# sigp/consensus-specs

Measured on AMD Instinct MI355X. Metric: BLS sig verifications/sec (whole node), higher is better.
Workload: dtype u32 (381-bit Montgomery, 14x28-bit limbs in u32 words); 1 GPU; C2: 65536 independent bls_verify deposit PoP checks per GPU (domain=3, 1/16 tampered); global_batch=65536, parallelism=dp1 (independent items, no collective), batches_in_flight=1, subgroup_policy=pyecc

## Files before the change

consensus-specs_amd/csrc/bls381_defs.hpp:

```cpp
#pragma once
#include <stddef.h>
#include <stdint.h>

#if defined(__HIP__)
#include <hip/hip_runtime.h>
#if defined(__HIP_DEVICE_COMPILE__)
#define BLS_PHASE() __builtin_amdgcn_sched_barrier(0)
#define BLS_ANY(c) (__builtin_amdgcn_ballot_w64((c)) != 0)
#else
#define BLS_PHASE() ((void)0)
#define BLS_ANY(c) (c)
#endif
#define BLS_HD __host__ __device__
#define BLS_INLINE __host__ __device__ __forceinline__
#define BLS_NOINLINE __host__ __device__ __attribute__((noinline))
#define BLS_DEV_INLINE __host__ __device__ __forceinline__
#define BLS_CONST __device__ __constant__ static constexpr
#else
#define BLS_PHASE() ((void)0)
#define BLS_ANY(c) (c)
#define BLS_HD
#define BLS_INLINE inline __attribute__((always_inline))
#define BLS_NOINLINE __attribute__((noinline))
#define BLS_DEV_INLINE inline
#define BLS_CONST static constexpr
#endif

namespace bls381 {

constexpr int FP_LIMBS = 14;
constexpr int FP_BITS = 28;
constexpr uint32_t FP_MASK = (1u << 28) - 1;
struct fp_t { uint32_t w[14]; };
struct fp2_t { fp_t c0, c1; };
template <class E> struct fp6_g { E c0, c1, c2; };
template <class E> struct fp12_g { fp6_g<E> c0, c1; };
using fp6_t = fp6_g<fp2_t>;
using fp12_t = fp12_g<fp2_t>;
struct fp2p_t { fp_t v; };

struct g1_jac { fp_t x, y, z; };
struct g2_jac { fp2_t x, y, z; };
struct g1_aff { fp_t x, y; };
struct g2_aff { fp2_t x, y; };

constexpr int KBLOCK = 128;
struct agg_chunk { uint32_t begin, end; };
constexpr int ML_STEPS = 68;
constexpr int ML_LC = 5;
constexpr size_t ML_L_WORDS_PER_ITEM = (size_t)ML_STEPS * ML_LC * FP_LIMBS * 2;
enum : uint32_t { SSZ_CHUNK = 1, SSZ_MERKLE = 2 };
constexpr int SSZ_STACK = 64;
constexpr int SSZ_PROG_MAX = 512;

}
```

consensus-specs_amd/csrc/bls381_field.hpp:

```cpp
#pragma once
#include "bls381_defs.hpp"
#include "bls381_consts.hpp"

namespace bls381 {

#if defined(BLS_COUNT_OPS) && !defined(__HIP_DEVICE_COMPILE__)
inline thread_local uint64_t g_fp_macs = 0;
#define BLS_COUNT_MACS(k) (g_fp_macs += (k))
#else
#define BLS_COUNT_MACS(k) ((void)0)
#endif
#if !defined(__HIP_DEVICE_COMPILE__) && !defined(__HIP__)
inline uint64_t g_inv_fallbacks = 0;
#define BLS_COUNT_INV_FALLBACK() (++g_inv_fallbacks)
#else
#define BLS_COUNT_INV_FALLBACK() ((void)0)
#endif

BLS_INLINE fp_t fp_zero() { fp_t r; for (int i = 0; i < 14; ++i) r.w[i] = 0; return r; }
BLS_INLINE fp_t fp_one() { return FP_ONE_M; }

BLS_INLINE void fp_carry(int32_t (&t)[14]) {
#pragma unroll
  for (int i = 0; i < 13; ++i) {
    t[i + 1] += t[i] >> 28;
    t[i] &= (int32_t)FP_MASK;
  }
}

template <int KMAX>
BLS_INLINE fp_t fp_reduce_lc(const uint32_t (&s)[14]) {
  static_assert(KMAX >= 1 && KMAX <= 8, "value bound");
  int32_t t[14];
  if (KMAX <= 2) {
    const uint32_t m = (int32_t)s[13] > (int32_t)Q2_LIMBS[13] ? ~0u : 0u;
#pragma unroll
    for (int i = 0; i < 14; ++i) t[i] = (int32_t)(s[i] - (Q2_LIMBS[i] & m));
  } else {
    const int32_t top = (int32_t)s[13] > 0 ? (int32_t)s[13] : 0;
    const uint32_t k = (uint32_t)(((uint64_t)(uint32_t)top * LC_DIV_MAGIC) >> 40);
#pragma unroll
    for (int i = 0; i < 14; ++i) t[i] = (int32_t)(s[i] + k * NQ2_LIMBS[i]);
  }
  fp_carry(t);
  if (BLS_ANY(t[13] >= (int32_t)Q2_LIMBS[13])) {
    int32_t e[14];
#pragma unroll
    for (int i = 0; i < 14; ++i) e[i] = t[i] - (int32_t)Q2_LIMBS[i];
    fp_carry(e);
    const bool ge = e[13] >= 0;
#pragma unroll
    for (int i = 0; i < 14; ++i) t[i] = ge ? e[i] : t[i];
  }
  fp_t r;
#pragma unroll
  for (int i = 0; i < 14; ++i) r.w[i] = (uint32_t)t[i];
  return r;
}

BLS_INLINE fp_t fp_add(const fp_t& a, const fp_t& b) {
  uint32_t s[14];
#pragma unroll
  for (int i = 0; i < 14; ++i) s[i] = a.w[i] + b.w[i];
  return fp_reduce_lc<2>(s);
}

BLS_INLINE fp_t fp_sub(const fp_t& a, const fp_t& b) {
  uint32_t s[14];
#pragma unroll
  for (int i = 0; i < 14; ++i) s[i] = a.w[i] + Q2B_LIMBS[i] - b.w[i];
  return fp_reduce_lc<2>(s);
}

BLS_INLINE fp_t fp_neg(const fp_t& a) {
  uint32_t s[14];
#pragma unroll
  for (int i = 0; i < 14; ++i) s[i] = Q2B_LIMBS[i] - a.w[i];
  return fp_reduce_lc<2>(s);
}

BLS_INLINE fp_t fp_dbl(const fp_t& a) {
  uint32_t s[14];
#pragma unroll
  for (int i = 0; i < 14; ++i) s[i] = a.w[i] << 1;
  return fp_reduce_lc<2>(s);
}

BLS_INLINE fp_t fp_add_sub(const fp_t& a, const fp_t& b, const fp_t& c) {
  uint32_t s[14];
#pragma unroll
  for (int i = 0; i < 14; ++i) s[i] = a.w[i] + b.w[i] + Q2B_LIMBS[i] - c.w[i];
  return fp_reduce_lc<3>(s);
}

BLS_INLINE fp_t fp_add3(const fp_t& a, const fp_t& b, const fp_t& c) {
  uint32_t s[14];
#pragma unroll
  for (int i = 0; i < 14; ++i) s[i] = a.w[i] + b.w[i] + c.w[i];
  return fp_reduce_lc<3>(s);
}

BLS_INLINE fp_t fp_sub2(const fp_t& a, const fp_t& b, const fp_t& c) {
  uint32_t s[14];
#pragma unroll
  for (int i = 0; i < 14; ++i) s[i] = a.w[i] + Q4B_LIMBS[i] - b.w[i] - c.w[i];
  return fp_reduce_lc<3>(s);
}

BLS_INLINE fp_t fp_3m2(const fp_t& X, const fp_t& x) {
  uint32_t s[14];
#pragma unroll
  for (int i = 0; i < 14; ++i) s[i] = 3u * X.w[i] + Q4B_LIMBS[i] - (x.w[i] << 1);
  return fp_reduce_lc<5>(s);
}
BLS_INLINE fp_t fp_3p2(const fp_t& X, const fp_t& x) {
  uint32_t s[14];
#pragma unroll
  for (int i = 0; i < 14; ++i) s[i] = 3u * X.w[i] + (x.w[i] << 1);
  return fp_reduce_lc<5>(s);
}
BLS_INLINE fp_t fp_3pm2(const fp_t& X, const fp_t& x, bool minus) {
  uint32_t s[14];
#pragma unroll
  for (int i = 0; i < 14; ++i) {
    const uint32_t x2 = x.w[i] << 1;
    s[i] = 3u * X.w[i] + (minus ? Q4B_LIMBS[i] - x2 : x2);
  }
  return fp_reduce_lc<5>(s);
}

BLS_INLINE fp_t fp_add_lazy(const fp_t& a, const fp_t& b) {
  fp_t r;
#pragma unroll
  for (int i = 0; i < 14; ++i) r.w[i] = a.w[i] + b.w[i];
  return r;
}

BLS_INLINE fp_t fp_reduce_once(const fp_t& s) {
  int32_t b[14];
#pragma unroll
  for (int i = 0; i < 14; ++i) b[i] = (int32_t)s.w[i] - (int32_t)Q_LIMBS[i];
  fp_carry(b);
  const bool neg = b[13] < 0;
  fp_t r;
#pragma unroll
  for (int i = 0; i < 14; ++i) r.w[i] = neg ? s.w[i] : (uint32_t)b[i];
  return r;
}

BLS_INLINE bool fp_is_zero(const fp_t& a) {
  uint32_t z = 0, e = 0;
#pragma unroll
  for (int i = 0; i < 14; ++i) { z |= a.w[i]; e |= a.w[i] ^ Q_LIMBS[i]; }
  return z == 0 || e == 0;
}

BLS_INLINE bool fp_eq(const fp_t& a, const fp_t& b) { return fp_is_zero(fp_sub(a, b)); }

BLS_INLINE fp_t fp_half(const fp_t& a) {
  const uint32_t odd = a.w[0] & 1u;
  int32_t s[14];
#pragma unroll
  for (int i = 0; i < 14; ++i) s[i] = (int32_t)(a.w[i] + (odd ? Q_LIMBS[i] : 0u));
  fp_carry(s);
  fp_t r;
#pragma unroll
  for (int i = 0; i < 13; ++i) r.w[i] = ((uint32_t)s[i] >> 1) | (((uint32_t)s[i + 1] & 1u) << 27);
  r.w[13] = (uint32_t)s[13] >> 1;
  return r;
}

BLS_INLINE fp_t fp_mul_body(const fp_t& a, const fp_t& b) {
  uint64_t T[28];
#pragma unroll
  for (int k = 0; k < 28; ++k) T[k] = 0;
#pragma unroll
  for (int i = 0; i < 14; ++i)
#pragma unroll
    for (int j = 0; j < 14; ++j) T[i + j] += (uint64_t)a.w[i] * b.w[j];
#pragma unroll
  for (int i = 0; i < 14; ++i) {
    const uint32_t m = ((uint32_t)T[i] * Q_INV28) & FP_MASK;
#pragma unroll
    for (int j = 0; j < 14; ++j) T[i + j] += (uint64_t)m * Q_LIMBS[j];
    T[i + 1] += T[i] >> 28;
  }
  fp_t r;
  uint64_t c = 0;
#pragma unroll
  for (int j = 0; j < 14; ++j) {
    const uint64_t v = T[14 + j] + c;
    r.w[j] = (uint32_t)v & FP_MASK;
    c = v >> 28;
  }
  return r;
}

BLS_INLINE fp_t fp_sqr_body(const fp_t& a) {
  uint64_t T[28];
  uint32_t a2[14];
#pragma unroll
  for (int k = 0; k < 28; ++k) T[k] = 0;
#pragma unroll
  for (int i = 0; i < 14; ++i) a2[i] = a.w[i] << 1;
#pragma unroll
  for (int i = 0; i < 14; ++i) {
    T[2 * i] += (uint64_t)a.w[i] * a.w[i];
#pragma unroll
    for (int j = i + 1; j < 14; ++j) T[i + j] += (uint64_t)a2[i] * a.w[j];
  }
#pragma unroll
  for (int i = 0; i < 14; ++i) {
    const uint32_t m = ((uint32_t)T[i] * Q_INV28) & FP_MASK;
#pragma unroll
    for (int j = 0; j < 14; ++j) T[i + j] += (uint64_t)m * Q_LIMBS[j];
    T[i + 1] += T[i] >> 28;
  }
  fp_t r;
  uint64_t c = 0;
#pragma unroll
  for (int j = 0; j < 14; ++j) {
    const uint64_t v = T[14 + j] + c;
    r.w[j] = (uint32_t)v & FP_MASK;
    c = v >> 28;
  }
  return r;
}

#if defined(__clang__)
typedef uint32_t fpv_t __attribute__((ext_vector_type(14)));
BLS_INLINE fpv_t fp_pack(const fp_t& a) {
  fpv_t v;
#pragma unroll
  for (int k = 0; k < 14; ++k) v[k] = a.w[k];
  return v;
}
BLS_INLINE fp_t fp_unpack(const fpv_t& v) {
  fp_t a;
#pragma unroll
  for (int k = 0; k < 14; ++k) a.w[k] = v[k];
  return a;
}
BLS_NOINLINE fpv_t fp_mul_call(fpv_t a, fpv_t b) { return fp_pack(fp_mul_body(fp_unpack(a), fp_unpack(b))); }
BLS_NOINLINE fpv_t fp_sqr_call(fpv_t a) { return fp_pack(fp_sqr_body(fp_unpack(a))); }
BLS_INLINE fp_t fp_mul(const fp_t& a, const fp_t& b) { return fp_unpack(fp_mul_call(fp_pack(a), fp_pack(b))); }
BLS_INLINE fp_t fp_sqr(const fp_t& a) { return fp_unpack(fp_sqr_call(fp_pack(a))); }
#else
BLS_NOINLINE fp_t fp_mul(fp_t a, fp_t b) { BLS_COUNT_MACS(392); return fp_mul_body(a, b); }
BLS_NOINLINE fp_t fp_sqr(fp_t a) { BLS_COUNT_MACS(301); return fp_sqr_body(a); }
#endif

BLS_INLINE fp_t fp_mul_small(const fp_t& a, int k) {
  if (k <= 8) {
    uint32_t s[14];
#pragma unroll
    for (int i = 0; i < 14; ++i) s[i] = (uint32_t)k * a.w[i];
    return fp_reduce_lc<8>(s);
  }
  fp_t r = a;
  fp_t acc = fp_zero();
  bool first = true;
  while (k) {
    if (k & 1) { acc = first ? r : fp_add(acc, r); first = false; }
    k >>= 1;
    if (k) r = fp_dbl(r);
  }
  return acc;
}

BLS_DEV_INLINE fp_t fp_pow_limbs(const fp_t& a, const uint32_t* e, int nbits) {
  fp_t r = FP_ONE_M;
  for (int i = nbits - 1; i >= 0; --i) {
    r = fp_sqr(r);
    if ((e[i >> 5] >> (i & 31)) & 1u) r = fp_mul(r, a);
  }
  return r;
}

BLS_HD inline fp_t fp_pow_qm3d4(const fp_t a) {
  const fp_t a2 = fp_sqr(a);
  const fp_t t1 = a, t3 = fp_mul(t1, a2), t5 = fp_mul(t3, a2), t7 = fp_mul(t5, a2);
  const fp_t t9 = fp_mul(t7, a2), t11 = fp_mul(t9, a2), t13 = fp_mul(t11, a2), t15 = fp_mul(t13, a2);
  fp_t r = FP_ONE_M;
  for (int k = 0; k < POW_QM3D4_NSTEPS; ++k) {
    for (int j = POW_QM3D4_SQR[k]; j > 0; --j) r = fp_sqr(r);
    switch (POW_QM3D4_DIG[k]) {
      case 1: r = fp_mul(r, t1); break;
      case 3: r = fp_mul(r, t3); break;
      case 5: r = fp_mul(r, t5); break;
      case 7: r = fp_mul(r, t7); break;
      case 9: r = fp_mul(r, t9); break;
      case 11: r = fp_mul(r, t11); break;
      case 13: r = fp_mul(r, t13); break;
      case 15: r = fp_mul(r, t15); break;
      default: break;
    }
  }
  return r;
}

BLS_HD inline fp_t fp_inv(const fp_t am);

BLS_DEV_INLINE bool fp_sqrt(fp_t& r, const fp_t& a) {
  r = fp_mul(fp_pow_qm3d4(a), a);
  return fp_eq(fp_sqr(r), a);
}

BLS_INLINE fp_t fp_to_mont(const fp_t& plain) { return fp_mul(plain, FP_R2); }
BLS_INLINE fp_t fp_from_mont(const fp_t& m) {
  fp_t one = fp_zero();
  one.w[0] = 1;
  return fp_reduce_once(fp_mul(m, one));
}

BLS_INLINE bool fp_plain_lt_q(const fp_t& a) {
  int32_t b[14];
#pragma unroll
  for (int i = 0; i < 14; ++i) b[i] = (int32_t)a.w[i] - (int32_t)Q_LIMBS[i];
  fp_carry(b);
  return b[13] < 0;
}

BLS_INLINE bool fp_plain_is_zero(const fp_t& a) {
  uint32_t z = 0;
#pragma unroll
  for (int i = 0; i < 14; ++i) z |= a.w[i];
  return z == 0;
}

BLS_INLINE bool fp_plain_gt(const fp_t& a, const fp_t& b) {
  int32_t d[14];
#pragma unroll
  for (int i = 0; i < 14; ++i) d[i] = (int32_t)b.w[i] - (int32_t)a.w[i];
  fp_carry(d);
  return d[13] < 0;
}

BLS_INLINE bool fp_plain_is_upper_half(const fp_t& y) {
  int32_t b[14];
#pragma unroll
  for (int i = 0; i < 14; ++i) b[i] = (int32_t)(2 * y.w[i]) - (int32_t)Q_LIMBS[i];
  fp_carry(b);
  return b[13] >= 0;
}

BLS_INLINE fp_t fp_plain_from_be48(const uint8_t* p) {
  uint32_t w[12];
#pragma unroll
  for (int i = 0; i < 12; ++i) {
    const uint8_t* b = p + 44 - 4 * i;
    w[i] = ((uint32_t)b[0] << 24) | ((uint32_t)b[1] << 16) | ((uint32_t)b[2] << 8) | b[3];
  }
  fp_t r;
#pragma unroll
  for (int k = 0; k < 14; ++k) {
    const int bit = 28 * k, wi = bit >> 5, sh = bit & 31;
    uint64_t v = (uint64_t)w[wi] >> sh;
    if (wi + 1 < 12) v |= (uint64_t)w[wi + 1] << (32 - sh);
    r.w[k] = (uint32_t)v & FP_MASK;
  }
  return r;
}

BLS_INLINE void fp_plain_to_be48(uint8_t* p, const fp_t& a) {
#pragma unroll
  for (int i = 0; i < 12; ++i) {
    const int bit = 32 * i, k = bit / 28, sh = bit % 28;
    uint64_t v = (uint64_t)a.w[k] >> sh;
    if (k + 1 < 14) v |= (uint64_t)a.w[k + 1] << (28 - sh);
    if (k + 2 < 14 && 56 - sh < 32) v |= (uint64_t)a.w[k + 2] << (56 - sh);
    const uint32_t w = (uint32_t)v;
    uint8_t* b = p + 44 - 4 * i;
    b[0] = (uint8_t)(w >> 24);
    b[1] = (uint8_t)(w >> 16);
    b[2] = (uint8_t)(w >> 8);
    b[3] = (uint8_t)w;
  }
}

// ... 658 lines not shown
```

consensus-specs_amd/csrc/bls381_pair.hpp:

```cpp
#pragma once
#include <hip/hip_runtime.h>

#ifndef BLS_WAVE_BALANCE
#define BLS_WAVE_BALANCE 2
#endif
#ifndef BLS_BALANCE_SHIFT
#define BLS_BALANCE_SHIFT 16
#endif
namespace bls381 {
__device__ __forceinline__ unsigned wave_slot() {
  return (unsigned)__builtin_amdgcn_s_getreg((31 << 11) | 4) & 1u;
}
__device__ __forceinline__ void wave_prio(unsigned x) {
  const unsigned hi = (unsigned)__builtin_amdgcn_readfirstlane((int)((x + wave_slot()) & 1u));
  if (hi) __builtin_amdgcn_s_setprio(2); else __builtin_amdgcn_s_setprio(0);
}
__device__ __forceinline__ bool wave_has_lds() {
  return ((unsigned)__builtin_amdgcn_s_getreg((31 << 11) | 6) >> 12) & 0x1ffu;
}
__device__ __forceinline__ unsigned balance_clock() {
  return (unsigned)(__builtin_amdgcn_s_memrealtime() >> BLS_BALANCE_SHIFT);
}
__device__ __forceinline__ void wave_balance(unsigned step) {
#if BLS_WAVE_BALANCE == 2
  if (!wave_has_lds()) wave_prio(balance_clock());
  else wave_prio(step);
#elif BLS_WAVE_BALANCE == 1
  wave_prio(step);
#else
  (void)step;
#endif
}
__device__ __forceinline__ void wave_balance_lds(unsigned step) {
#if BLS_WAVE_BALANCE
  wave_prio(step);
#else
  (void)step;
#endif
}
__device__ __forceinline__ void wave_balance_call() {
#if BLS_WAVE_BALANCE == 2
  if (!wave_has_lds()) wave_prio(balance_clock());
#endif
}
}
#if BLS_WAVE_BALANCE && !defined(BLS_FE_STEP)
#define BLS_FE_STEP(j) ::bls381::wave_balance((unsigned)(j))
#endif
#include "bls381_hash.hpp"
#include "bls381_pairing.hpp"

namespace bls381 {

__device__ __forceinline__ bool pr_odd() { return (threadIdx.x & 1u) != 0; }

enum : int {
  DPP_SWAP = 0xB1,
  DPP_EVEN = 0xA0,
  DPP_ODD = 0xF5,
};

template <int CTRL>
__device__ __forceinline__ uint32_t pr_dpp(uint32_t x) {
  return (uint32_t)__builtin_amdgcn_mov_dpp((int)x, CTRL, 0xF, 0xF, false);
}
template <int CTRL>
__device__ __forceinline__ fp_t pr_dpp(const fp_t& a) {
  fp_t r;
#pragma unroll
  for (int k = 0; k < FP_LIMBS; ++k) r.w[k] = pr_dpp<CTRL>(a.w[k]);
  return r;
}
__device__ __forceinline__ bool pr_both(bool b) { return (pr_dpp<DPP_SWAP>((uint32_t)b) & (uint32_t)b) != 0; }

__device__ __forceinline__ fp_t fp_sel(bool c, const fp_t& a, const fp_t& b) {
  fp_t r;
#pragma unroll
  for (int k = 0; k < FP_LIMBS; ++k) r.w[k] = c ? a.w[k] : b.w[k];
  return r;
}

__device__ __forceinline__ fp_t fp2p_mul_body(const fp_t& a, const fp_t& b) {
  const bool odd = pr_odd();
  const fp_t ao = pr_dpp<DPP_SWAP>(a);
  const fp_t b0 = pr_dpp<DPP_EVEN>(b);
  const fp_t b1 = pr_dpp<DPP_ODD>(b);
  uint32_t w[14];
#pragma unroll
  for (int k = 0; k < 14; ++k) w[k] = odd ? b1.w[k] : Q8S_LIMBS[k] - b1.w[k];
  uint64_t T[28];
#pragma unroll
  for (int k = 0; k < 28; ++k) T[k] = 0;
#pragma unroll
  for (int i = 0; i < 14; ++i)
#pragma unroll
    for (int j = 0; j < 14; ++j) {
      T[i + j] += (uint64_t)a.w[i] * b0.w[j];
      T[i + j] += (uint64_t)ao.w[i] * w[j];
    }
  return fp_redc_wide(T);
}

__device__ __forceinline__ fp_t fp2p_sqr_body(const fp_t& a) {
  const bool odd = pr_odd();
  const fp_t ao = pr_dpp<DPP_SWAP>(a);
  fp_t x, y;
#pragma unroll
  for (int k = 0; k < 14; ++k) {
    x.w[k] = ao.w[k] + (odd ? ao.w[k] : a.w[k]);
    y.w[k] = odd ? a.w[k] : a.w[k] + Q8S_LIMBS[k] - ao.w[k];
  }
  return fp_mul_body(x, y);
}

#define BLS_FP2_CALL __device__ __attribute__((noinline))
BLS_FP2_CALL fpv_t fp2p_mul_call(fpv_t a, fpv_t b) {
  return fp_pack(fp2p_mul_body(fp_unpack(a), fp_unpack(b)));
}
BLS_FP2_CALL fpv_t fp2p_sqr_call(fpv_t a) {
  return fp_pack(fp2p_sqr_body(fp_unpack(a)));
}

__device__ __forceinline__ fp2p_t pr_make(const fp_t& v) { fp2p_t r; r.v = v; return r; }

template <> BLS_INLINE fp2p_t e2_zero<fp2p_t>() { return pr_make(fp_zero()); }
template <> BLS_INLINE fp2p_t e2_one<fp2p_t>() { return pr_make(fp_sel(pr_odd(), fp_zero(), FP_ONE_M)); }
template <> BLS_INLINE fp2p_t e2_k<fp2p_t>(const fp2_t& k) { return pr_make(fp_sel(pr_odd(), k.c1, k.c0)); }

__device__ __forceinline__ fp2p_t fp2_add(const fp2p_t& a, const fp2p_t& b) { return pr_make(fp_add(a.v, b.v)); }
__device__ __forceinline__ fp2p_t fp2_sub(const fp2p_t& a, const fp2p_t& b) { return pr_make(fp_sub(a.v, b.v)); }
__device__ __forceinline__ fp2p_t fp2_neg(const fp2p_t& a) { return pr_make(fp_neg(a.v)); }
__device__ __forceinline__ fp2p_t fp2_dbl(const fp2p_t& a) { return pr_make(fp_dbl(a.v)); }
__device__ __forceinline__ fp2p_t fp2_half(const fp2p_t& a) { return pr_make(fp_half(a.v)); }
__device__ __forceinline__ fp2p_t fp2_add_lazy(const fp2p_t& a, const fp2p_t& b) { return pr_make(fp_add_lazy(a.v, b.v)); }
__device__ __forceinline__ fp2p_t fp2_mul_fp(const fp2p_t& a, const fp_t& s) { return pr_make(fp_mul(a.v, s)); }
__device__ __forceinline__ fp2p_t fp2_mul_small(const fp2p_t& a, int k) { return pr_make(fp_mul_small(a.v, k)); }
__device__ __forceinline__ fp2p_t fp2_conj(const fp2p_t& a) { return pr_make(fp_sel(pr_odd(), fp_neg(a.v), a.v)); }
__device__ __forceinline__ fp2p_t fp2_mul_xi(const fp2p_t& a) {
  const bool odd = pr_odd();
  const fp_t ao = pr_dpp<DPP_SWAP>(a.v);
  uint32_t s[14];
#pragma unroll
  for (int i = 0; i < 14; ++i) s[i] = a.v.w[i] + (odd ? ao.w[i] : Q2B_LIMBS[i] - ao.w[i]);
  return pr_make(fp_reduce_lc<2>(s));
}
__device__ __forceinline__ fp2p_t fp2_add_mul_xi(const fp2p_t& a, const fp2p_t& b) {
  const bool odd = pr_odd();
  const fp_t bo = pr_dpp<DPP_SWAP>(b.v);
  uint32_t s[14];
#pragma unroll
  for (int i = 0; i < 14; ++i) s[i] = a.v.w[i] + b.v.w[i] + (odd ? bo.w[i] : Q2B_LIMBS[i] - bo.w[i]);
  return pr_make(fp_reduce_lc<3>(s));
}
__device__ __forceinline__ fp2p_t fp2_sub2(const fp2p_t& a, const fp2p_t& b, const fp2p_t& c) {
  return pr_make(fp_sub2(a.v, b.v, c.v));
}
__device__ __forceinline__ fp2p_t fp2_3m2(const fp2p_t& X, const fp2p_t& x) { return pr_make(fp_3m2(X.v, x.v)); }
__device__ __forceinline__ fp2p_t fp2_3p2(const fp2p_t& X, const fp2p_t& x) { return pr_make(fp_3p2(X.v, x.v)); }
__device__ __forceinline__ fp2p_t fp2_3pm2(const fp2p_t& X, const fp2p_t& x, bool minus) {
  return pr_make(fp_3pm2(X.v, x.v, minus));
}
__device__ __forceinline__ fp2p_t fp2_mul(const fp2p_t& a, const fp2p_t& b) {
  wave_balance_call();
  return pr_make(fp_unpack(fp2p_mul_call(fp_pack(a.v), fp_pack(b.v))));
}
__device__ __forceinline__ fp2p_t fp2_sqr(const fp2p_t& a) {
  wave_balance_call();
  return pr_make(fp_unpack(fp2p_sqr_call(fp_pack(a.v))));
}
__device__ __forceinline__ bool fp2_is_zero(const fp2p_t& a) { return pr_both(fp_is_zero(a.v)); }
__device__ __forceinline__ bool fp2_eq(const fp2p_t& a, const fp2p_t& b) { return pr_both(fp_eq(a.v, b.v)); }

__device__ __forceinline__ cyc_bc<fp2p_t> cyc_csqr_lazy(const cyc_bc<fp2p_t>& g) {
  const bool p = pr_odd();
  cyc_bc<fp2p_t> r;
  {
    const fp_t e4 = pr_dpp<DPP_EVEN>(g.g4.v), o4 = pr_dpp<DPP_ODD>(g.g4.v);
    const fp_t e5 = pr_dpp<DPP_EVEN>(g.g5.v), o5 = pr_dpp<DPP_ODD>(g.g5.v);
    r.g2 = pr_make(fp_6p2(lz_xi_mul(p, e4, o4, e5, o5), g.g2.v));
    r.g3 = pr_make(fp_3m2(lz_sqr_xisqr(p, e4, o4, e5, o5), g.g3.v));
  }
  const fp_t e2 = pr_dpp<DPP_EVEN>(g.g2.v), o2 = pr_dpp<DPP_ODD>(g.g2.v);
  const fp_t e3 = pr_dpp<DPP_EVEN>(g.g3.v), o3 = pr_dpp<DPP_ODD>(g.g3.v);
  r.g4 = pr_make(fp_3m2(lz_sqr_xisqr(p, e2, o2, e3, o3), g.g4.v));
  r.g5 = pr_make(fp_6p2(lz_mul(p, e2, o2, e3, o3), g.g5.v));
  return r;
}

#ifndef BLS_INV_PAIR
#define BLS_INV_PAIR 1
#endif
__device__ inline fp_t fp_inv_pair(const fp_t am) {
  const bool odd = pr_odd();
  uint32_t w[12];
  fp_plain_to_words(w, fp_reduce_once(am));
  uint32_t z = 0;
#pragma unroll
  for (int i = 0; i < 12; ++i) z |= w[i];
  if (z == 0) return fp_zero();
  int32_t A[INV_L], X[INV_L], Y[INV_L], U[INV_L], V[INV_L];
  inv_to_l30(A, w);
#pragma unroll
  for (int i = 0; i < INV_L; ++i) {
    X[i] = odd ? Q_L30[i] : A[i];
    Y[i] = odd ? A[i] : Q_L30[i];
    U[i] = 0;
    V[i] = 0;
  }
  if (odd) V[0] = 1; else U[0] = 1;
  for (int round = 0; round < 26; ++round) {
    int t = 2;
    uint32_t top = 0;
#pragma unroll
    for (int i = 2; i < INV_L; ++i) {
      const uint32_t c = (uint32_t)(X[i] | Y[i]);
      if (c) { t = i; top = c; }
    }
    const int bl = top ? 32 - __builtin_clz(top) : 2;
    uint32_t x2 = 0, x1 = 0, x0 = 0, y2 = 0, y1 = 0, y0 = 0;
#pragma unroll
    for (int i = 2; i < INV_L; ++i) {
      const bool s = i == t;
      x2 = s ? (uint32_t)X[i] : x2; x1 = s ? (uint32_t)X[i - 1] : x1; x0 = s ? (uint32_t)X[i - 2] : x0;
      y2 = s ? (uint32_t)Y[i] : y2; y1 = s ? (uint32_t)Y[i - 1] : y1; y0 = s ? (uint32_t)Y[i - 2] : y0;
    }
    const uint32_t a2 = odd ? y2 : x2, a1 = odd ? y1 : x1, a0 = odd ? y0 : x0;
    const uint32_t b2 = odd ? x2 : y2, b1 = odd ? x1 : y1, b0 = odd ? x0 : y0;
    const uint32_t al0 = (uint32_t)(odd ? Y[0] : X[0]), bl0 = (uint32_t)(odd ? X[0] : Y[0]);
    const uint32_t al1 = (uint32_t)(odd ? Y[1] : X[1]), bl1 = (uint32_t)(odd ? X[1] : Y[1]);
    const uint32_t al2 = (uint32_t)(odd ? Y[2] : X[2]), bl2 = (uint32_t)(odd ? X[2] : Y[2]);
    const uint64_t wa = ((uint64_t)a2 << 31) | ((uint64_t)a1 << 1) | (a0 >> 29);
    const uint64_t wb = ((uint64_t)b2 << 31) | ((uint64_t)b1 << 1) | (b0 >> 29);
    uint64_t xa = ((wa >> (bl - 1)) << 30) | al0;
    uint64_t xb = ((wb >> (bl - 1)) << 30) | bl0;
    if (t == 2 && bl <= 2) {
      xa = al0 | ((uint64_t)al1 << 30) | ((uint64_t)al2 << 60);
      xb = bl0 | ((uint64_t)bl1 << 30) | ((uint64_t)bl2 << 60);
    }
    int32_t f0 = 1, g0 = 0, f1 = 0, g1 = 1;
#pragma unroll 10
    for (int j = 0; j < 30; ++j) {
      const bool od = (xa & 1) != 0;
      const bool sw = od && xa < xb;
      const uint64_t ta = sw ? xb : xa, tb = sw ? xa : xb;
      const int32_t tf0 = sw ? f1 : f0, tg0 = sw ? g1 : g0, tf1 = sw ? f0 : f1, tg1 = sw ? g0 : g1;
      xa = (od ? ta - tb : ta) >> 1;
      xb = tb;
      f0 = od ? tf0 - tf1 : tf0;
      g0 = od ? tg0 - tg1 : tg0;
      f1 = tf1 + tf1;
      g1 = tg1 + tg1;
    }
    int32_t cX = odd ? g1 : f0, cY = odd ? f1 : g0;
// ... 197 lines not shown
```

consensus-specs_amd/csrc/host_check.cpp:

```cpp
#include <cstring>
#include <map>
#include <string>
#include <thread>
#include <vector>

#include "bls381_hash.hpp"
#include "bls381_pairing.hpp"
#include "bls381_plan.hpp"
#include "bls381_ssz.hpp"

using namespace bls381;

namespace {
fp_t ld(const uint8_t* p) { return fp_to_mont(fp_plain_from_be48(p)); }
void st(uint8_t* p, const fp_t& a) { fp_plain_to_be48(p, fp_from_mont(a)); }
fp2_t ld2(const uint8_t* p) { fp2_t r; r.c0 = ld(p); r.c1 = ld(p + 48); return r; }
void st2(uint8_t* p, const fp2_t& a) { st(p, a.c0); st(p + 48, a.c1); }
fp12_t ld12(const uint8_t* p) {
  fp12_t r;
  r.c0.c0 = ld2(p); r.c0.c1 = ld2(p + 96); r.c0.c2 = ld2(p + 192);
  r.c1.c0 = ld2(p + 288); r.c1.c1 = ld2(p + 384); r.c1.c2 = ld2(p + 480);
  return r;
}
void st12(uint8_t* p, const fp12_t& a) {
  st2(p, a.c0.c0); st2(p + 96, a.c0.c1); st2(p + 192, a.c0.c2);
  st2(p + 288, a.c1.c0); st2(p + 384, a.c1.c1); st2(p + 480, a.c1.c2);
}
aff_t<fp_t> ldg1(const uint8_t* p) { aff_t<fp_t> a; a.x = ld(p); a.y = ld(p + 48); return a; }
aff_t<fp2_t> ldg2(const uint8_t* p) { aff_t<fp2_t> a; a.x = ld2(p); a.y = ld2(p + 96); return a; }
}

extern "C" {

void hc_fp_lc_raw(int op, const uint32_t* a, const uint32_t* b, const uint32_t* c, uint32_t* o) {
  fp_t x, y, z, r;
  for (int i = 0; i < 14; ++i) { x.w[i] = a[i]; y.w[i] = b[i]; z.w[i] = c[i]; }
  switch (op) {
    case 0: r = fp_add(x, y); break;
    case 1: r = fp_sub(x, y); break;
    case 2: r = fp_neg(x); break;
    case 3: r = fp_dbl(x); break;
    case 4: r = fp_add_sub(x, y, z); break;
    case 5: r = fp_add3(x, y, z); break;
    case 6: r = fp_sub2(x, y, z); break;
    case 7: r = fp_3m2(x, y); break;
    case 8: r = fp_3p2(x, y); break;
    default: r = fp_mul_small(x, op - 8); break;
  }
  for (int i = 0; i < 14; ++i) o[i] = r.w[i];
}

void hc_fp_mul(const uint8_t* a, const uint8_t* b, uint8_t* o) { st(o, fp_mul(ld(a), ld(b))); }
void hc_fp_add(const uint8_t* a, const uint8_t* b, uint8_t* o) { st(o, fp_add(ld(a), ld(b))); }
void hc_fp_sub(const uint8_t* a, const uint8_t* b, uint8_t* o) { st(o, fp_sub(ld(a), ld(b))); }
void hc_fp_half(const uint8_t* a, uint8_t* o) { st(o, fp_half(ld(a))); }
void hc_fp_inv(const uint8_t* a, uint8_t* o) { st(o, fp_inv(ld(a))); }
void hc_fp_inv_xgcd(const uint8_t* a, uint8_t* o) { st(o, fp_inv_xgcd(ld(a))); }
uint64_t hc_inv_fallbacks() { return g_inv_fallbacks; }
int hc_fp_sqrt(const uint8_t* a, uint8_t* o) {
  fp_t r;
  const bool ok = fp_sqrt(r, ld(a));
  st(o, r);
  return ok;
}
int hc_fp_legendre(const uint8_t* a) { return fp_legendre(ld(a)); }
void hc_fp_mont_mul_raw(const uint8_t* a, const uint8_t* b, uint8_t* o) {
  fp_plain_to_be48(o, fp_mul(fp_plain_from_be48(a), fp_plain_from_be48(b)));
}

void hc_fp2_mul(const uint8_t* a, const uint8_t* b, uint8_t* o) { st2(o, fp2_mul(ld2(a), ld2(b))); }
void hc_fp2_sqr(const uint8_t* a, uint8_t* o) { st2(o, fp2_sqr(ld2(a))); }
void hc_fp2_inv(const uint8_t* a, uint8_t* o) { st2(o, fp2_inv(ld2(a))); }
int hc_fp2_sqrt_select(const uint8_t* a, uint8_t* o) {
  fp2_t r;
  if (!fp2_sqrt(r, ld2(a))) return 0;
  st2(o, g2_select_root(r));
  return 1;
}

static fp2_t ldraw2(const uint8_t* p) { fp2_t r; r.c0 = fp_plain_from_be48(p); r.c1 = fp_plain_from_be48(p + 48); return r; }
static void straw2(uint8_t* p, const fp2_t& a) { fp_plain_to_be48(p, a.c0); fp_plain_to_be48(p + 48, a.c1); }
void hc_fp2_mul_lazy_raw(const uint8_t* x, const uint8_t* y, const uint8_t* z, const uint8_t* u, uint8_t* o) {
  straw2(o, fp2_mul(fp2_add_lazy(ldraw2(x), ldraw2(y)), fp2_add_lazy(ldraw2(z), ldraw2(u))));
}

void hc_cyc_csqr_raw(const uint8_t* in, uint8_t* out) {
  cyc_bc<fp2_t> g;
  g.g2 = ldraw2(in); g.g3 = ldraw2(in + 96); g.g4 = ldraw2(in + 192); g.g5 = ldraw2(in + 288);
  const cyc_bc<fp2_t> r = cyc_csqr(g);
  straw2(out, r.g2); straw2(out + 96, r.g3); straw2(out + 192, r.g4); straw2(out + 288, r.g5);
}

}
namespace {
fp_t rw(const uint32_t*& p) { fp_t r; for (int i = 0; i < 14; ++i) r.w[i] = *p++; return r; }
fp2_t rw2(const uint32_t*& p) { fp2_t r; r.c0 = rw(p); r.c1 = rw(p); return r; }
fp12_t rw12(const uint32_t*& p) {
  fp12_t r;
  r.c0.c0 = rw2(p); r.c0.c1 = rw2(p); r.c0.c2 = rw2(p); r.c1.c0 = rw2(p); r.c1.c1 = rw2(p); r.c1.c2 = rw2(p);
  return r;
}
void ww(uint32_t*& o, const fp_t& a) { for (int i = 0; i < 14; ++i) *o++ = a.w[i]; }
void ww2(uint32_t*& o, const fp2_t& a) { ww(o, a.c0); ww(o, a.c1); }
void ww12(uint32_t*& o, const fp12_t& a) {
  ww2(o, a.c0.c0); ww2(o, a.c0.c1); ww2(o, a.c0.c2); ww2(o, a.c1.c0); ww2(o, a.c1.c1); ww2(o, a.c1.c2);
}
jac_t<fp2_t> rwjac(const uint32_t*& p) { jac_t<fp2_t> r; r.x = rw2(p); r.y = rw2(p); r.z = rw2(p); return r; }
aff_t<fp2_t> rwaff(const uint32_t*& p) { aff_t<fp2_t> r; r.x = rw2(p); r.y = rw2(p); return r; }
int wwjac(uint32_t*& o, const jac_t<fp2_t>& a) { ww2(o, a.x); ww2(o, a.y); ww2(o, a.z); return jac_is_inf(a) ? 1 : 0; }
}
extern "C" {

int hc_raw_fp2(int op, const uint32_t* in, uint64_t aux, uint32_t* out) {
  switch (op) {
    case 0: { const fp2_t a = rw2(in), b = rw2(in); ww2(out, fp2_mul(a, b)); return 0; }
    case 1: ww2(out, fp2_sqr(rw2(in))); return 0;
    case 2: ww2(out, fp2_inv(rw2(in))); return 0;
    default: {
      cyc_bc<fp2_t> g;
      g.g2 = rw2(in); g.g3 = rw2(in); g.g4 = rw2(in); g.g5 = rw2(in);
      for (uint64_t j = 0; j < aux; ++j) g = cyc_csqr(g);
      ww2(out, g.g2); ww2(out, g.g3); ww2(out, g.g4); ww2(out, g.g5);
      return 0;
    }
  }
}
int hc_raw_fp12(int op, const uint32_t* in, uint64_t aux, uint32_t* out) {
  const fp12_t f = op == 9 ? fp12_one<fp2_t>() : rw12(in);
  switch (op) {
    case 0: ww12(out, fp12_mul(f, rw12(in))); return 0;
    case 1: ww12(out, fp12_sqr(f)); return 0;
    case 2: ww12(out, fp12_cyclotomic_sqr(f)); return 0;
    case 3: { const fp2_t c0 = rw2(in), c1 = rw2(in), c2 = rw2(in); ww12(out, fp12_mul_by_line(f, c0, c1, c2)); return 0; }
    case 4: ww12(out, fp12_frob(f, (int)aux)); return 0;
    case 5: ww12(out, fp12_inv(f)); return 0;
    case 6: ww12(out, final_exp(f)); return 0;
    case 7: ww12(out, cyc_exp_x<fp2_t, 1>(f)); return 0;
    case 8: ww12(out, cyc_exp_x_gs(f)); return 0;
    default: {
      cyc_bc<fp2_t> g;
      g.g2 = rw2(in); g.g3 = rw2(in); g.g4 = rw2(in); g.g5 = rw2(in);
      ww12(out, cyc_decompress(g, rw2(in)));
      return 0;
    }
  }
}
int hc_raw_g2(int op, const uint32_t* in, uint64_t aux, uint32_t* out) {
  switch (op) {
    case 0: return wwjac(out, jac_dbl(rwjac(in)));
    case 1: { const jac_t<fp2_t> p = rwjac(in); return wwjac(out, jac_add_aff(p, rwaff(in))); }
    case 2: { const jac_t<fp2_t> p = rwjac(in); return wwjac(out, jac_add(p, rwjac(in))); }
    case 3: return wwjac(out, g2_psi_jac(rwjac(in)));
    case 4: return wwjac(out, jac_mul_u64(rwaff(in), aux));
    default: return wwjac(out, g2_mul_bp(rwaff(in)));
  }
}
int hc_raw_miller(int n, const uint32_t* in, uint32_t* out) {
  aff_t<fp2_t> Q[2];
  g1_line_pre P[2];
  if (n < 1 || n > 2) return -1;
  for (int k = 0; k < n; ++k) {
    Q[k] = rwaff(in);
    aff_t<fp_t> p; p.x = rw(in); p.y = rw(in);
    P[k] = g1_prepare(p);
  }
  bool degen = false;
  ww12(out, n == 1 ? miller_loop_n<1>(Q, P, degen) : miller_loop_n<2>(Q, P, degen));
  return degen ? 1 : 0;
}

void hc_fp12_mul(const uint8_t* a, const uint8_t* b, uint8_t* o) { st12(o, fp12_mul(ld12(a), ld12(b))); }
void hc_fp12_sqr(const uint8_t* a, uint8_t* o) { st12(o, fp12_sqr(ld12(a))); }
void hc_fp12_inv(const uint8_t* a, uint8_t* o) { st12(o, fp12_inv(ld12(a))); }
void hc_fp12_frob(const uint8_t* a, int p, uint8_t* o) { st12(o, fp12_frob(ld12(a), p)); }
void hc_fp12_cyc_sqr(const uint8_t* a, uint8_t* o) { st12(o, fp12_cyclotomic_sqr(ld12(a))); }
void hc_fp12_mul_by_line(const uint8_t* f, const uint8_t* c0, const uint8_t* c1, const uint8_t* c2, uint8_t* o) {
  st12(o, fp12_mul_by_line(ld12(f), ld2(c0), ld2(c1), ld2(c2)));
}
void hc_final_exp(const uint8_t* a, uint8_t* o) { st12(o, final_exp(ld12(a))); }
int hc_final_exp_check(const uint8_t* a, int fb) {
  return fb ? final_exp_check<fp2_t, 1>(ld12(a)) : final_exp_check<fp2_t, 0>(ld12(a));
}

int hc_g1_decompress(const uint8_t* b48, uint8_t* aff96, int lax) {
  aff_t<fp_t> a;
  const int s = g1_decompress(a, b48, lax != 0);
  if (s == PT_OK) { st(aff96, a.x); st(aff96 + 48, a.y); }
  return s;
}
int hc_g2_decompress(const uint8_t* b96, uint8_t* aff192, int lax) {
  aff_t<fp2_t> a;
  const int s = g2_decompress(a, b96, lax != 0);
  if (s == PT_OK) { st2(aff192, a.x); st2(aff192 + 96, a.y); }
  return s;
}
void hc_g1_compress_aff(const uint8_t* aff96, uint8_t* b48) { g1_compress(b48, jac_from_aff(ldg1(aff96))); }
void hc_g2_compress_aff(const uint8_t* aff192, uint8_t* b96) { g2_compress_aff(b96, ldg2(aff192)); }
int hc_g1_in_subgroup(const uint8_t* aff96) { return g1_in_subgroup(ldg1(aff96)); }
int hc_g2_in_subgroup(const uint8_t* aff192) { return g2_in_subgroup(ldg2(aff192)); }

int hc_hash_to_g2(const uint8_t* msg, uint32_t mlen, const uint8_t* dom8, uint8_t* aff192, uint8_t* comp96) {
  aff_t<fp2_t> c;
  const int trials = hash_to_g2_candidate(c, msg, mlen, dom8);
  aff_t<fp2_t> h;
  if (!jac_to_aff(h, g2_mul_cofactor(c))) return -2;
  st2(aff192, h.x); st2(aff192 + 96, h.y);
  g2_compress_aff(comp96, h);
  return trials;
}
void hc_sha256(const uint8_t* msg, uint32_t len, uint8_t* out32) {
  uint32_t d[8];
  sha256(d, msg, len);
  for (int i = 0; i < 8; ++i) {
    out32[4 * i] = (uint8_t)(d[i] >> 24); out32[4 * i + 1] = (uint8_t)(d[i] >> 16);
    out32[4 * i + 2] = (uint8_t)(d[i] >> 8); out32[4 * i + 3] = (uint8_t)d[i];
  }
}

int hc_miller_loop(int n, const uint8_t* q192, const uint8_t* p96, uint8_t* o576) {
  aff_t<fp2_t> Q[4];
  g1_line_pre P[4];
  if (n < 1 || n > 4) return -1;
  for (int k = 0; k < n; ++k) { Q[k] = ldg2(q192 + 192 * k); P[k] = g1_prepare(ldg1(p96 + 96 * k)); }
  fp12_t f;
  bool degen = false;
  switch (n) {
    case 1: f = miller_loop_n<1>(Q, P, degen); break;
    case 2: f = miller_loop_n<2>(Q, P, degen); break;
    case 3: f = miller_loop_n<3>(Q, P, degen); break;
    default: f = miller_loop_n<4>(Q, P, degen); break;
  }
  st12(o576, f);
  return degen ? 1 : 0;
}

static bool g1_in(const aff_t<fp_t>& a) { return g1_in_subgroup(a); }
static bool g2_in(const aff_t<fp2_t>& a) { return g2_in_subgroup(a); }

static int verify_pairs(int np, const aff_t<fp2_t>* Q, const aff_t<fp_t>* Pa) {
  fp12_t f = fp12_one<fp2_t>();
  for (int k = 0; k < np; ++k) {
    bool degen = false;
    g1_line_pre P = g1_prepare(Pa[k]);
    f = fp12_mul(f, miller_loop_n<1>(&Q[k], &P, degen));
    if (degen) return 0;
  }
  return fp12_is_one(final_exp(f)) ? 1 : 0;
}

int hc_verify(const uint8_t* pk48, const uint8_t* msg, uint32_t mlen, const uint8_t* sig96, const uint8_t* dom8,
              int strict) {
  aff_t<fp_t> P;
  aff_t<fp2_t> S;
  const int sp = g1_decompress(P, pk48, !strict);
  const int ss = g2_decompress(S, sig96, !strict);
  if (sp == PT_BAD || ss == PT_BAD) return 0;
  if (strict && ((sp == PT_OK && !g1_in(P)) || (ss == PT_OK && !g2_in(S)))) return 0;
  aff_t<fp2_t> Q[2];
  aff_t<fp_t> Pa[2];
  int np = 0;
  if (ss == PT_OK) {
    Q[np] = S;
    Pa[np].x = G1_VGEN_X_M;
    Pa[np].y = G1_VGEN_NEGY_M;
// ... 285 lines not shown
```

Baseline: 2.474 million verifications/s.

## Switch Montgomery mul/sqr to product-scanning columns with interleaved reduction

```diff
diff --git a/consensus-specs_amd/csrc/bls381_defs.hpp b/consensus-specs_amd/csrc/bls381_defs.hpp
--- a/consensus-specs_amd/csrc/bls381_defs.hpp
+++ b/consensus-specs_amd/csrc/bls381_defs.hpp
@@ -24,6 +24,12 @@
 #define BLS_NOINLINE __attribute__((noinline))
 #define BLS_DEV_INLINE inline
 #define BLS_CONST static constexpr
+#endif
+
+#if defined(__clang__)
+#define BLS_KEEP_ORDER(x) __builtin_annotation((x), "bls381.order")
+#else
+#define BLS_KEEP_ORDER(x) (x)
 #endif
 
 namespace bls381 {
diff --git a/consensus-specs_amd/csrc/bls381_field.hpp b/consensus-specs_amd/csrc/bls381_field.hpp
--- a/consensus-specs_amd/csrc/bls381_field.hpp
+++ b/consensus-specs_amd/csrc/bls381_field.hpp
@@ -170,61 +170,48 @@
   return r;
 }
 
-BLS_INLINE fp_t fp_mul_body(const fp_t& a, const fp_t& b) {
-  uint64_t T[28];
-#pragma unroll
-  for (int k = 0; k < 28; ++k) T[k] = 0;
-#pragma unroll
-  for (int i = 0; i < 14; ++i)
-#pragma unroll
-    for (int j = 0; j < 14; ++j) T[i + j] += (uint64_t)a.w[i] * b.w[j];
-#pragma unroll
-  for (int i = 0; i < 14; ++i) {
-    const uint32_t m = ((uint32_t)T[i] * Q_INV28) & FP_MASK;
-#pragma unroll
-    for (int j = 0; j < 14; ++j) T[i + j] += (uint64_t)m * Q_LIMBS[j];
-    T[i + 1] += T[i] >> 28;
-  }
+BLS_INLINE uint64_t fp_mac(uint64_t acc, uint32_t x, uint32_t y) { return BLS_KEEP_ORDER(acc + (uint64_t)x * y); }
+
+template <class F>
+BLS_INLINE fp_t fp_mont_columns(const F& col) {
+  uint32_t m[14];
   fp_t r;
   uint64_t c = 0;
 #pragma unroll
-  for (int j = 0; j < 14; ++j) {
-    const uint64_t v = T[14 + j] + c;
-    r.w[j] = (uint32_t)v & FP_MASK;
-    c = v >> 28;
-  }
-  return r;
+  for (int k = 0; k < 27; ++k) {
+    uint64_t acc = col(k, c);
+#pragma unroll
+    for (int i = (k > 13 ? k - 13 : 0); i < k && i < 14; ++i) acc = fp_mac(acc, m[i], Q_LIMBS[k - i]);
+    if (k < 14) {
+      m[k] = ((uint32_t)acc * Q_INV28) & FP_MASK;
+      acc = fp_mac(acc, m[k], Q_LIMBS[0]);
+    } else {
+      r.w[k - 14] = (uint32_t)acc & FP_MASK;
+    }
+    c = acc >> 28;
+  }
+  r.w[13] = (uint32_t)c & FP_MASK;
+  return r;
+}
+
+BLS_INLINE fp_t fp_mul_body(const fp_t& a, const fp_t& b) {
+  return fp_mont_columns([&](int k, uint64_t acc) {
+#pragma unroll
+    for (int i = (k > 13 ? k - 13 : 0); i <= k && i < 14; ++i) acc = fp_mac(acc, a.w[i], b.w[k - i]);
+    return acc;
+  });
 }
 
 BLS_INLINE fp_t fp_sqr_body(const fp_t& a) {
-  uint64_t T[28];
   uint32_t a2[14];
 #pragma unroll
-  for (int k = 0; k < 28; ++k) T[k] = 0;
-#pragma unroll
   for (int i = 0; i < 14; ++i) a2[i] = a.w[i] << 1;
-#pragma unroll
-  for (int i = 0; i < 14; ++i) {
-    T[2 * i] += (uint64_t)a.w[i] * a.w[i];
-#pragma unroll
-    for (int j = i + 1; j < 14; ++j) T[i + j] += (uint64_t)a2[i] * a.w[j];
-  }
-#pragma unroll
-  for (int i = 0; i < 14; ++i) {
-    const uint32_t m = ((uint32_t)T[i] * Q_INV28) & FP_MASK;
-#pragma unroll
-    for (int j = 0; j < 14; ++j) T[i + j] += (uint64_t)m * Q_LIMBS[j];
-    T[i + 1] += T[i] >> 28;
-  }
-  fp_t r;
-  uint64_t c = 0;
-#pragma unroll
-  for (int j = 0; j < 14; ++j) {
-    const uint64_t v = T[14 + j] + c;
-    r.w[j] = (uint32_t)v & FP_MASK;
-    c = v >> 28;
-  }
-  return r;
+  return fp_mont_columns([&](int k, uint64_t acc) {
+#pragma unroll
+    for (int i = (k > 13 ? k - 13 : 0); 2 * i < k; ++i) acc = fp_mac(acc, a2[i], a.w[k - i]);
+    if ((k & 1) == 0) acc = fp_mac(acc, a.w[k / 2], a.w[k / 2]);
+    return acc;
+  });
 }
 
 #if defined(__clang__)
diff --git a/consensus-specs_amd/csrc/bls381_pair.hpp b/consensus-specs_amd/csrc/bls381_pair.hpp
--- a/consensus-specs_amd/csrc/bls381_pair.hpp
+++ b/consensus-specs_amd/csrc/bls381_pair.hpp
@@ -88,17 +88,14 @@
   uint32_t w[14];
 #pragma unroll
   for (int k = 0; k < 14; ++k) w[k] = odd ? b1.w[k] : Q8S_LIMBS[k] - b1.w[k];
-  uint64_t T[28];
-#pragma unroll
-  for (int k = 0; k < 28; ++k) T[k] = 0;
-#pragma unroll
-  for (int i = 0; i < 14; ++i)
-#pragma unroll
-    for (int j = 0; j < 14; ++j) {
-      T[i + j] += (uint64_t)a.w[i] * b0.w[j];
-      T[i + j] += (uint64_t)ao.w[i] * w[j];
-    }
-  return fp_redc_wide(T);
+  return fp_mont_columns([&](int k, uint64_t acc) {
+#pragma unroll
+    for (int i = (k > 13 ? k - 13 : 0); i <= k && i < 14; ++i) {
+      acc = fp_mac(acc, a.w[i], b0.w[k - i]);
+      acc = fp_mac(acc, ao.w[i], w[k - i]);
+    }
+    return acc;
+  });
 }
 
 __device__ __forceinline__ fp_t fp2p_sqr_body(const fp_t& a) {
diff --git a/consensus-specs_amd/csrc/host_check.cpp b/consensus-specs_amd/csrc/host_check.cpp
--- a/consensus-specs_amd/csrc/host_check.cpp
+++ b/consensus-specs_amd/csrc/host_check.cpp
@@ -110,6 +110,11 @@
 int wwjac(uint32_t*& o, const jac_t<fp2_t>& a) { ww2(o, a.x); ww2(o, a.y); ww2(o, a.z); return jac_is_inf(a) ? 1 : 0; }
 }
 extern "C" {
+
+void hc_raw_fp(int op, const uint32_t* in, uint32_t* out) {
+  const fp_t a = rw(in);
+  ww(out, op == 0 ? fp_mul(a, rw(in)) : fp_sqr(a));
+}
 
 int hc_raw_fp2(int op, const uint32_t* in, uint64_t aux, uint32_t* out) {
   switch (op) {
```

Result: faster. 2.534 million verifications/s (median of 6 runs) (+2.4%).
